# TimD1/vcfdist

Hardware: AMD Instinct MI355X
Metric: supercluster-alignments/sec (higher is better)
Workload: dtype int32; 1 GPU; wgs_synth; superclusters_per_gpu=1000000, span_dist=lognormal(median 20, sigma 1.2) clip [4,10000]

## Files before the change

### vcfdist_amd/csrc/pr_api.hip

```cpp
#include <hip/hip_runtime.h>
#include <hip/hip_ext.h>
#include <dlfcn.h>

#include <algorithm>
#include <atomic>
#include <chrono>
#include <cstdarg>
#include <cstdio>
#include <cstdlib>
#include <cstring>
#include <condition_variable>
#include <deque>
#include <functional>
#include <mutex>
#include <string>
#include <thread>
#include <tuple>
#include <unordered_map>
#include <unordered_set>
#include <vector>

#include "../../include/vcfdist_pr.h"
#include "pr_device.h"
#include "pr_plan.h"
// ... 734 lines not shown
        const int64_t D1_FLOOR = int64_t(4) << 20;
        const int64_t slack = 64 * 5 * int64_t(len_max + 1);
        const int64_t in_all = 2 * in_chunk_max + slack, log_all = 2 * log_max + 160 * int64_t((n_short_max + 63) / 64) + 160 * int64_t(len_max + 1);
        h->d1_in_cap = std::min(in_all, std::max(int64_t(D1_SHARE * double(in_all)), D1_FLOOR + slack));
        h->d1_log_cap = std::min(log_all, std::max(int64_t(D1_SHARE * double(log_all)), D1_FLOOR + slack));
        const int64_t cap_ip = std::min<int64_t>(n_short_max, std::max<int64_t>(4096, (n_short_max / 4 + 3) & ~int64_t(3)));
        h->d1_wave_cap = int32_t((cap_ip + 63) / 64);
        h->d1_fail_cap = int32_t(n_short_max + n_short_max / 8 + 1024);
        h->soft_alloc = true;
        int rc = dev_alloc(h, &h->d_d1_hdr, size_t(h->d1_wave_cap));
        if (!rc) rc = dev_alloc(h, &h->d_d1_in, size_t(h->d1_in_cap));
        if (!rc) rc = dev_alloc(h, &h->d_d1_log, size_t(h->d1_log_cap));
        if (!rc) rc = dev_alloc(h, &h->d_d1_fail, size_t(h->d1_fail_cap));
        if (!rc) rc = dev_alloc(h, &h->d_d1_info, 16);
        if (!rc) rc = dev_alloc(h, &h->d_d1_blk, size_t(h->d1_fail_cap / 256 + 8));
        h->soft_alloc = false;
        if (rc) {
            if (h->debug) fprintf(stderr, "[vpr] distance-1 lane level: no room for its blocks (%.2f GB), the level is off for this batch\n",
                                  double(h->d1_in_cap) * 4e-9 + double(h->d1_log_cap) * 16e-9);
            h->d_d1_hdr = nullptr; h->d_d1_in = nullptr; h->d_d1_log = nullptr; h->d_d1_fail = nullptr; h->d_d1_info = nullptr; h->d_d1_blk = nullptr;
            h->err.clear();
            (void)hipGetLastError();
        } else {
            HIPCHK(h, hipMemsetAsync(h->d_d1_info, 0, 64, h->stream));
        }
    }
    for (size_t ci = 0; ci < P.chunks.size(); ci++) {
        const Chunk &ch = P.chunks[ci];
        const int64_t n_short = ch.count - ch.n_long;
        if (n_short <= 0) continue;
        hipLaunchKernelGGL(k_prep_zl, dim3(unsigned((n_short + 63) / 64)), dim3(256), 0, h->stream, h->dB, h->d_descs,
                           P.d_work + ch.work_off + ch.n_long, int(n_short), h->d_zl_hdr + h->zl_wave0[ci], h->d_zl_in);
    }
    HIPCHK(h, hipGetLastError());
    if (h->debug) fprintf(stderr, "[vpr] zero-distance lane level: %zu waves, %.2f GB position words, %.2f GB log\n", n_waves,
                          double(in_words) * 4e-9, double(log_max) * 16e-9);
    return VPR_OK;
}

// ... 288 lines not shown
            VPRCHK(dev_alloc(h, &D.cand2_r[q], ref_len));
            VPRCHK(dev_alloc(h, &D.fk_q[q], hap_len[q]));
            VPRCHK(dev_alloc(h, &D.fk_r[q], ref_len));
            VPRCHK(dev_alloc(h, &D.bk_q[q], hap_len[q]));
            VPRCHK(dev_alloc(h, &D.bk_r[q], ref_len));
            VPRCHK(dev_alloc(h, &D.vs_ref[q], ref_len));
            VPRCHK(dev_alloc(h, &D.fk4_q[q], hap_len[q]));
            VPRCHK(dev_alloc(h, &D.fk4_r[q], ref_len));
            VPRCHK(dev_alloc(h, &D.tk[q], hap_len[2 + q]));
            VPRCHK(dev_alloc(h, &D.tj[q], hap_len[2 + q] + 8));
            VPRCHK(dev_alloc(h, &D.wk_q[q], hap_len[q]));
            VPRCHK(dev_alloc(h, &D.wk_r[q], ref_len));
            VPRCHK(dev_alloc(h, &D.wk_t[q], hap_len[2 + q]));
            VPRCHK(dev_alloc(h, &D.xb_q[q], hap_len[q]));
            VPRCHK(dev_alloc(h, &D.xb_r[q], ref_len));
            HIPCHK(h, hipMemsetAsync(D.cand_q[q], 0xff, std::max<int64_t>(hap_len[q], 1) * sizeof(int4), h->stream));
            HIPCHK(h, hipMemsetAsync(D.cand_r[q], 0xff, std::max<int64_t>(ref_len, 1) * sizeof(int4), h->stream));
            HIPCHK(h, hipMemsetAsync(D.cand2_q[q], 0xff, std::max<int64_t>(hap_len[q], 1) * sizeof(int4), h->stream));
            HIPCHK(h, hipMemsetAsync(D.cand2_r[q], 0xff, std::max<int64_t>(ref_len, 1) * sizeof(int4), h->stream));
        }
        lap("  inputs: reference arrays, constants' blocks");
        VPRCHK(dev_alloc(h, &h->d_err, 1));
        HIPCHK(h, hipMemsetAsync(h->d_err, 0, 4, h->stream));
        if (!h->ev_offsets) HIPCHK(h, hipEventCreateWithFlags(&h->ev_offsets, hipEventDisableTiming));
        HIPCHK(h, hipEventRecord(h->ev_offsets, h->stream));
        return VPR_OK;
    }

    int generate() {
        if (!h->gen_src) return VPR_OK;
// ... 45 lines not shown
    }

    template <typename K, typename... A>
    void query_planes(K kernel, A... tail) {
        for (int q = 0; q < 2; q++) {
            if (hap_len[q] > 0) hipLaunchKernelGGL(kernel, blocks(hap_len[q]), dim3(256), 0, h->stream, D, q, 0, hap_len[q], tail...);
            if (ref_len > 0) hipLaunchKernelGGL(kernel, blocks(ref_len), dim3(256), 0, h->stream, D, q, 1, ref_len, tail...);
        }
    }

    int prep_kernels() {
        for (hipEvent_t &e : ev_prep) HIPCHK(h, hipEventCreate(&e));
        HIPCHK(h, hipEventRecord(ev_prep[0], h->stream));
        if (n > 0) hipLaunchKernelGGL(k_prep_scof, dim3(unsigned((n + 255) / 256), 5), dim3(256), 0, h->stream, D);
        query_planes(k_prep_cand, h->d_err);
        query_planes(k_prep_pack);
        lap("  prep: scof, cand, pack");
        for (int s = 0; s < 4; s++)
            if (hap_len[s] > 0)
                hipLaunchKernelGGL(k_prep_ins, blocks(hap_len[s]), dim3(256), 0, h->stream, D, s, hap_len[s]);
        if (n > 0) hipLaunchKernelGGL(k_prep_suffix, dim3((n + 4 * SUFFIX_SC_PER_WAVE - 1) / (4 * SUFFIX_SC_PER_WAVE), 6), dim3(256), 0, h->stream, D);
        int2 *pd = nullptr;
        VPRCHK(pin_array(h, &pd, size_t(std::max(n, 1)) * 4));
        for (int s = 0; s < 4; s++) {
            h->hp_dspan[s] = pd + size_t(s) * size_t(n);
            if (n > 0) HIPCHK(h, hipMemcpyAsync(h->hp_dspan[s], D.dspan[s], size_t(n) * sizeof(int2), hipMemcpyDeviceToHost, h->stream));
        }
        lap("  prep: ins, suffix, spans");
        query_planes(k_prep_xb);
        for (int s = 0; s < 2; s++)
            if (hap_len[2 + s] > 0) hipLaunchKernelGGL(k_prep_tj, blocks(hap_len[2 + s]), dim3(256), 0, h->stream, D, s, hap_len[2 + s]);
        for (int w = 0; w < 6; w++) {
            const int64_t npos = w < 2 ? hap_len[w] : (w < 4 ? ref_len : hap_len[w - 2]);
            if (npos > 0) hipLaunchKernelGGL(k_prep_q16, blocks(npos), dim3(256), 0, h->stream, D, w, npos);
            if (npos > 0) hipLaunchKernelGGL(k_prep_wk, blocks(npos), dim3(256), 0, h->stream, D, w, npos);
        }
        HIPCHK(h, hipEventRecord(ev_prep[1], h->stream));
        return VPR_OK;
    }

    int batch_pass() {
        h->descs.set(b, h->var_off);
        h->ed_max_len = -1;
        na = h->descs.size();
        for (int s = 0; s < 4; s++) sec_total += 2 * b->var_off[s][n];
        sec_total += 16 * int64_t(n);
        const bool plan_pass = lv0 <= LV_Q16 && !(h->cfg.flags & VPR_CFG_HAP_DEDUP) && n > 0;
        const int LLT = h->long_lt;
        h->p0 = vpr_handle::Plan0Pass();
        if (plan_pass) h->level.resize(size_t(n) * 4);
// ... 1205 lines not shown
    void ordered_fails(const int32_t *list, int32_t nc, int32_t *out, int32_t *cnt, const int32_t *n_dev, hipStream_t ks) {
        const int nb = (nc + 255) / 256;
        hipLaunchKernelGGL(k_fails_count, dim3(nb), dim3(256), 0, ks, list, nc, h->d_outs, h->d_d1_blk, 1, n_dev);
        hipLaunchKernelGGL(k_fails_scan, dim3(1), dim3(FAILS_SCAN_NT), 0, ks, h->d_d1_blk, nb, cnt);
        hipLaunchKernelGGL(k_fails_scatter, dim3(nb), dim3(256), 0, ks, list, nc, h->d_outs, h->d_d1_blk, out, 1, n_dev);
    }

    int enqueue_d1(const int32_t *list, const int32_t *n_dev, int32_t cap, int32_t n_all, hipStream_t ks, int ph, int ztag) {
        const int nw = (cap + 63) / 64;
        vpr_launch_stat ls;
        memset(&ls, 0, sizeof(ls));
        ls.threads = 64; ls.cells_per_thread = 1; ls.n_units = cap;
        int rc = VPR_OK;
        if (ph == 1) {
            rc = timed(0, ls, ks, "k_prep_d1", [&] {
                hipLaunchKernelGGL(k_d1_hdr, dim3(nw), dim3(64), 0, ks, h->d_descs, list, n_dev, cap, h->d_outs, h->d_d1_hdr);
                hipLaunchKernelGGL(k_d1_scan, dim3(1), dim3(D1_SCAN_NT), 0, ks, h->d_d1_hdr, nw, h->d1_in_cap, h->d1_log_cap, h->d_d1_info);
                hipLaunchKernelGGL(k_prep_d1, dim3(nw), dim3(256), 0, ks, h->dB, h->d_descs, list, n_dev, cap, h->d_outs, h->d_d1_hdr, h->d_d1_in);
            });
            if (rc) return rc;
            rc = timed(1, ls, ks, "k_one_lane", [&] {
                hipLaunchKernelGGL(k_one_lane, dim3(nw), dim3(64), 0, ks, h->d_descs, list, n_dev, cap, h->d_d1_hdr, h->d_d1_in, h->d_d1_log,
                                   h->d_outs, reinterpret_cast<PathEnt *>(h->plan0.arena), (h->cfg.flags & VPR_CFG_KEEP_PATHS) ? 1 : 0, h->d_d1_info,
                                   std::max(1, h->lane_prio_rows / 4));
                hipLaunchKernelGGL(k_fwd_band_finish, dim3((cap + 255) / 256), dim3(256), 0, ks, list, cap, h->d_outs, D1_TAG, n_dev);
            });
            if (rc) return rc;
            ordered_fails(list, n_all, h->d_d1_fail, h->d_d1_info + 2, n_dev, ks);
        } else if (ph == 4) {
            ls.cells_per_thread = 3;
            rc = timed(3, ls, ks, "k_one_tail", [&] {
                hipLaunchKernelGGL(k_one_tail, dim3(nw), dim3(64), 0, ks, h->dB, h->d_descs, list, n_dev, cap, h->d_d1_hdr, h->d_d1_in, h->d_d1_log,
                                   h->d_outs, reinterpret_cast<PathEnt *>(h->plan0.arena), (h->cfg.flags & VPR_CFG_KEEP_PATHS) ? 1 : 0, h->d_d1_info,
// ... 399 lines not shown
                for (int ph = 1; ph <= 4; ph <<= 1) {
                    if ((rc = enqueue_part(P0, P0.d_work, ch.work_off + n_long, n_short, P0.lv, s_short, 1, n_long, false,
                                           ch.part_cells[1], ch.part_in[1], ch.part_dense[1], -1, ph))) return rc;
                    if (ph == 1) post_flag(1, s_short);
                    if (ph == 2 && (rc = collect_part(1, short_list, n_short, s_short))) return rc;
                }
            }
            if (inplace) {
                zl_wave0 = h->zl_wave0[ci];
                zl_rows = ch.part_rows[1];
                const int32_t *n_dev = h->d_cnt + 1;
                const int ztag = LV_TAG[LV_Z];
                HIPCHK(h, hipMemsetAsync(h->d_cnt + SLOT_IP, 0, 4, s_short));
                const bool d1 = h->d_d1_hdr != nullptr && cap_ip <= h->d1_wave_cap * 64;
                const int32_t n_all1 = n_short + n_short / 16 + 64;
                if (d1) HIPCHK(h, hipMemsetAsync(h->d_d1_info + 2, 0, 4, s_short));
                hipStream_t s_cred = h->side_credit ? h->cls_stream[7] : s_short;
                for (int ph = 1; ph <= 4; ph <<= 1) {
                    if (ph != 4 || s_cred == s_short) {
                        if ((rc = enqueue_part(P0, P0.d_work, ch.work_off + n_long, n_short, LV_Z, s_short, 1, n_long, false,
                                               ch.part_cells[1], ch.part_in[1], ch.part_dense[1], -1, ph))) return rc;
                        if (d1 && (rc = enqueue_d1(h->d_fail + n_long, n_dev, cap_ip, n_all1, s_short, ph, ztag))) return rc;
                    }
                    if (ph == 1 && s_cred != s_short) {
                        HIPCHK(h, hipEventRecord(h->ev_cred[0], s_short));
                        HIPCHK(h, hipStreamWaitEvent(s_cred, h->ev_cred[0], 0));
                        if ((rc = enqueue_part(P0, P0.d_work, ch.work_off + n_long, n_short, LV_Z, s_cred, 1, n_long, false,
                                               ch.part_cells[1], ch.part_in[1], ch.part_dense[1], -1, 4))) return rc;
                        if (d1 && (rc = enqueue_d1(h->d_fail + n_long, n_dev, cap_ip, n_all1, s_cred, 4, ztag))) return rc;
                        HIPCHK(h, hipEventRecord(h->ev_cred[1], s_cred));
                    }
// ... 505 lines not shown
```

### vcfdist_amd/csrc/pr_d1.hip

```cpp
#ifndef PR_D1_HIP_
#define PR_D1_HIP_

#define D1_TAG 9
#define D1_CLEAN ZL_CLEAN_REJECT

#define GE_ALIVE 1u
#define GE_MAT 2u
#define GE_SWP 4u
#define GE_PSLOT_SHIFT 3
#define GE_SUB 32u
#define GE_SUB_SHIFT 6
#define GE_INS 256u
#define GE_INS_SHIFT 9
#define GE_DEL 2048u
#define GE_DEL_SHIFT 12
#define GE_TP 16384u
#define GE_BWD 32768u

#define MV_SWP_R 0
#define MV_MAT 1
#define MV_SUB 2
#define MV_INS 3
#define MV_DEL 4
#define MV_SWP_Q 5

__global__ void __launch_bounds__(64) k_d1_hdr(const AlnDesc *__restrict__ descs, const int32_t *__restrict__ list,
                                               const int32_t *__restrict__ n_dev, int n_cap, const AlnOut *__restrict__ outs,
                                               ZlWave *__restrict__ hdr) {
    const int w = blockIdx.x, lane = threadIdx.x;
    const int n = min(*n_dev, n_cap);
    const int wi = w * 64 + lane;
    const int a = wi < n ? list[wi] : -1;
    int lq = 0, lr = 0, lt = 0;
    if (a >= 0 && outs[a].exit_min == D1_CLEAN) {
        const AlnDesc *d = descs + a;
        lq = d->Lq; lr = d->Lr; lt = d->Lt;
    }
#pragma unroll
    for (int o = 32; o; o >>= 1) {
        lq = max(lq, __shfl_xor(lq, o)); lr = max(lr, __shfl_xor(lr, o)); lt = max(lt, __shfl_xor(lt, o));
    }
    if (lane == 0) {
        ZlWave W;
        W.in_off = 0; W.log_off = 0; W.mq = lq; W.mr = lr; W.mt = lt; W.pad = 0;
        hdr[w] = W;
    }
}

#define D1_SCAN_NT 256
__global__ void __launch_bounds__(D1_SCAN_NT) k_d1_scan(ZlWave *__restrict__ hdr, int n_waves, int64_t in_cap, int64_t log_cap,
                                                  int32_t *__restrict__ info) {
    __shared__ int64_t s_in[D1_SCAN_NT], s_log[D1_SCAN_NT];
    __shared__ int s_used, s_drop;
    const int tid = threadIdx.x;
    if (tid == 0) { s_used = 0; s_drop = 0; }
    const int per = (n_waves + D1_SCAN_NT - 1) / D1_SCAN_NT;
    const int b = min(n_waves, tid * per), e = min(n_waves, b + per);
    int64_t si = 0, sl = 0;
    for (int k = b; k < e; k++) {
        const ZlWave W = hdr[k];
        if (W.mt > 0) { si += 64 * (2 * int64_t(W.mq) + 2 * int64_t(W.mr) + W.mt); sl += 160 * (int64_t(W.mt) + 1); }
    }
    s_in[tid] = si; s_log[tid] = sl;
    __syncthreads();
    for (int o = 1; o < D1_SCAN_NT; o <<= 1) {
        const int64_t ai = tid >= o ? s_in[tid - o] : 0, al = tid >= o ? s_log[tid - o] : 0;
        __syncthreads();
        s_in[tid] += ai; s_log[tid] += al;
        __syncthreads();
    }
    int64_t oi = s_in[tid] - si, ol = s_log[tid] - sl;
    int used = 0, drop = 0;
    for (int k = b; k < e; k++) {
        ZlWave W = hdr[k];
        if (W.mt <= 0) continue;
        const int64_t ni = 64 * (2 * int64_t(W.mq) + 2 * int64_t(W.mr) + W.mt), nl = 160 * (int64_t(W.mt) + 1);
        if (oi + ni > in_cap || ol + nl > log_cap) { W.mq = W.mr = W.mt = 0; drop++; }
        else { W.in_off = oi; W.log_off = ol; used++; }
        oi += ni; ol += nl;
        hdr[k] = W;
    }
    if (used) atomicAdd(&s_used, used);
    if (drop) atomicAdd(&s_drop, drop);
    __syncthreads();
    if (tid == 0) { info[0] = s_used; info[1] = s_drop; }
}

__global__ void __launch_bounds__(256) k_prep_d1(DevBatch B, const AlnDesc *__restrict__ descs, const int32_t *__restrict__ list,
                                                 const int32_t *__restrict__ n_dev, int n_cap, const AlnOut *__restrict__ outs,
                                                 const ZlWave *__restrict__ hdr, uint32_t *__restrict__ zin) {
    __shared__ uint32_t tile[64][65];
    __shared__ int64_t s_qo[64], s_ro[64], s_to[64];
    __shared__ int32_t s_lq[64], s_lr[64], s_lt[64];
    __shared__ uint8_t s_qs[64], s_ts[64];
    const int w = blockIdx.x;
    const ZlWave H = hdr[w];
    if (H.mt <= 0) return;
    const int n_list = min(*n_dev, n_cap);
    const int lane = threadIdx.x & 63, sub = threadIdx.x >> 6;
    if (threadIdx.x < 64) {
        const int wi = w * 64 + lane;
        int a = wi < n_list ? list[wi] : -1;
        if (a >= 0 && outs[a].exit_min != D1_CLEAN) a = -1;
        if (a >= 0) {
            const AlnDesc *d = descs + a;
            s_qo[lane] = d->q_off; s_ro[lane] = d->r_off; s_to[lane] = d->t_off;
            s_lq[lane] = d->Lq; s_lr[lane] = d->Lr; s_lt[lane] = d->Lt;
            s_qs[lane] = uint8_t(d->qs); s_ts[lane] = uint8_t(d->ts);
        } else {
            s_qo[lane] = s_ro[lane] = s_to[lane] = 0;
            s_lq[lane] = s_lr[lane] = s_lt[lane] = 0;
            s_qs[lane] = 0; s_ts[lane] = 2;
        }
    }
    __syncthreads();
    auto flagbits = [](int f) -> uint32_t { return ((f & PV) ? ZW_PV : 0u) | ((f & PB) ? ZW_PB : 0u) | ((f & PE) ? ZW_PE : 0u); };
    uint32_t *out = zin + H.in_off;
    for (int arr = 0; arr < 5; arr++) {
        const int pl = arr >> 1;
        const bool src_words = (arr & 1) && arr < 4;
        const int mlen = pl == 0 ? H.mq : (pl == 1 ? H.mr : H.mt);
        for (int x0 = 0; x0 < mlen; x0 += 64) {
            const int x = x0 + lane;
#pragma unroll 16
            for (int k = 0; k < 16; k++) {
                const int l = sub * 16 + k;
                const int qs = s_qs[l], ts = s_ts[l];
                const int Lr = s_lr[l];
                const int len = pl == 0 ? s_lq[l] : (pl == 1 ? Lr : s_lt[l]);
                uint32_t v = src_words ? 0u : 0x7f0000u;
                if (x < len) {
                    const int64_t ro = s_ro[l];
                    if (src_words) {
                        const int4 c = pl == 0 ? B.cand_q[qs][s_qo[l] + x] : B.cand_r[qs][ro + x];
                        v = uint32_t(c.x >= 0 ? c.x + 1 : 0) | (c.z >= 0 ? 0xffff0000u : (uint32_t(c.y >= 0 ? c.y + 1 : 0) << 16));
                    } else {
                        const int slot = pl == 2 ? ts : qs;
                        const int64_t o = (pl == 0 ? s_qo[l] : (pl == 1 ? ro : s_to[l])) + x;
                        const uint8_t *seq = pl == 1 ? B.ref_seq : B.hap_seq[slot];
                        const int2 *wk = pl == 0 ? B.wk_q[qs] : (pl == 1 ? B.wk_r[qs] : B.wk_t[ts - 2]);
                        const int2 k2 = wk[o];
                        const int p = k2.x, f = pl == 1 ? int(B.ref_flag[qs][o]) : (k2.y & 0xff);
                        const uint32_t ins = ((k2.y >> 8) & ((1 << qs) | (1 << ts))) ? ZW_INS : 0u;
                        v = uint32_t((p + 1) & 0xffff) | (uint32_t(seq[o] & 0x7f) << 16) | flagbits(f) | ins;
                        if (pl == 0 && x > 0 && ((p != wk[o - 1].x + 1) || (f & PB))) v |= ZW_TP;
                        (void)Lr;
                    }
                }
                tile[lane][l] = v;
            }
            __syncthreads();
            const int rows = min(64, mlen - x0);
            for (int r = sub; r < rows; r += 4) out[int64_t(x0 + r) * 64 + lane] = tile[r][lane];
            __syncthreads();
        }
        out += int64_t(mlen) * 64;
    }
}

__global__ void __launch_bounds__(64, 3) k_one_lane(const AlnDesc *__restrict__ descs, const int32_t *__restrict__ list,
                                                    const int32_t *__restrict__ n_dev, int n_cap, const ZlWave *__restrict__ hdr,
                                                    const uint32_t *__restrict__ zin, uint4 *__restrict__ zlog,
                                                    AlnOut *__restrict__ outs, PathEnt *__restrict__ paths, int keep_paths,
                                                    int32_t *__restrict__ info, int prio_rows) {
    const int w = blockIdx.x, lane = threadIdx.x;
    const ZlWave H = hdr[w];
    if (H.mt <= 0) return;
    if (H.mt >= prio_rows) __builtin_amdgcn_s_setprio(2);
    const int n_list = min(*n_dev, n_cap);
    const int wi = w * 64 + lane;
    int a_ = wi < n_list ? list[wi] : -1;
    if (a_ >= 0 && outs[a_].exit_min != D1_CLEAN) a_ = -1;
// ... 586 lines not shown
```

### vcfdist_amd/csrc/pr_device.h

```cpp
#ifndef PR_DEVICE_H_
#define PR_DEVICE_H_
#include <hip/hip_runtime.h>
#include <stdint.h>

#define F_INS 1
#define F_DEL 2
#define F_MAT 4
#define F_SUB 8
#define F_SWP 16
#define F_CHOICE_SHIFT 5
#define F_TIE 128
#define F_CHOICE_MASK (0x60u | F_SUB)
__host__ __device__ __forceinline__ uint32_t f_choice_bits(int rank) { return (uint32_t(rank & 3) << F_CHOICE_SHIFT) | (uint32_t(rank >> 2) << 3); }
__host__ __device__ __forceinline__ int f_choice_of(uint32_t f) { return int(((f >> F_CHOICE_SHIFT) & 3u) | ((f >> 1) & 4u)); }
__host__ __device__ __forceinline__ uint32_t f_diag(uint32_t f) { return f & (F_MAT | (F_SUB & ~(f >> 1))); }
__host__ __device__ __forceinline__ uint32_t rank_bits(int rank) { return (uint32_t(rank & 3) << 1) | (uint32_t(rank >> 2) << 4); }
__host__ __device__ __forceinline__ int rank_of(uint32_t bits) { return int(((bits >> 1) & 3u) | ((bits >> 2) & 4u)); }
#define F_SWP_KEY_MASK (F_SWP | F_CHOICE_MASK)
__host__ __device__ __forceinline__ uint32_t f_swp_key(int rank) { return F_SWP | f_choice_bits(rank); }
#define SWAP_SOURCES_MAX 8
#define F_KEEP 0xe0

#define PV 1
#define PB 2
// ... 30 lines not shown
    int2 *fk_r[2];
    int32_t *bk_q[2];
    int32_t *bk_r[2];
    int32_t *vs_hap[4];
    int32_t *vs_ref[2];
    int2 *xb_q[2];
    int2 *xb_r[2];
    int2 *dspan[4];
    int4 *fk4_q[2];
    int4 *fk4_r[2];
    int2 *tk[2];
    uint16_t *tj[2];
    int2 *wk_q[2];
    int2 *wk_r[2];
    int2 *wk_t[2];
};
#define FK_MULTI (1 << 30)
#define FK_NONE24 0xffffff

struct AlnDesc {
    int64_t q_off, t_off, r_off;
    int32_t Lq, Lt, Lr;
    int32_t qs, ts;
    int32_t sc, aln;
    int32_t pitch[2];
    int64_t mat_off[2];
    int64_t path_off;
    int64_t sec_off;
    int32_t sec_cap;
    int32_t path_cap;
// ... 131 lines not shown
```

### vcfdist_amd/csrc/pr_host.h

```cpp
#ifndef PR_HOST_H_
#define PR_HOST_H_
#include <hip/hip_runtime.h>
#include <hip/hip_ext.h>

#include <algorithm>
#include <atomic>
#include <chrono>
#include <cstdarg>
#include <cstdio>
#include <cstdlib>
#include <cstring>
#include <condition_variable>
#include <deque>
#include <functional>
#include <mutex>
#include <string>
#include <thread>
#include <tuple>
#include <unordered_map>
#include <unordered_set>
#include <vector>

#include "../../include/vcfdist_pr.h"
#include "pr_device.h"
// ... 270 lines not shown
    EdJob *d_jobs = nullptr; int32_t jobs_cap = 0; int32_t *d_njobs = nullptr;
    uint32_t *d_err = nullptr;
    int32_t *d_fail = nullptr, *d_cnt = nullptr;
    int4 *d_tie_list = nullptr, *hp_tie_list = nullptr; int32_t tie_list_cap = 0;
    int32_t *hp_flag = nullptr; int32_t flag_seq = 0;
    int32_t *d_tie_cnt = nullptr, *hp_tie_cnt = nullptr;
    hipEvent_t ev_spec = nullptr;
    TieJob *hp_tie_jobs = nullptr; size_t tie_jobs_cap = 0;
    int4 *d_tie_dec = nullptr; int64_t tie_dec_cap = 0;
    int32_t *d_tie_ndec = nullptr;
    std::vector<int32_t> plan0_pos;
    ZlWave *d_zl_hdr = nullptr; uint32_t *d_zl_in = nullptr; uint4 *d_zl_log = nullptr;
    std::vector<int64_t> zl_wave0;
    ZlWave *d_d1_hdr = nullptr; uint32_t *d_d1_in = nullptr; uint4 *d_d1_log = nullptr; int32_t *d_d1_fail = nullptr, *d_d1_info = nullptr;
    int32_t *d_d1_blk = nullptr;
    hipEvent_t ev_offsets = nullptr;
    hipEvent_t ev_cred[2] = {nullptr, nullptr};
    bool side_credit = true;
    struct Plan0Pass {
        bool valid = false, bad = false;
        int64_t part_cells[2] = {0, 0}, part_in[2] = {0, 0}, part_dense[2] = {0, 0}, part_rows[2] = {0, 0}, need128 = 0, need_max = 0;
        std::vector<std::pair<int64_t, int32_t>> big;
    } p0;
    int64_t d1_in_cap = 0, d1_log_cap = 0;
    int32_t d1_wave_cap = 0, d1_fail_cap = 0;
    int32_t d1_max_rows = 256;
    std::vector<ZlWave> zl_hdr_host;
    int32_t long_lt = LONG_LT;
    const vpr_variants *gen_src = nullptr;
    uint8_t *d_ctg_seq = nullptr; const uint8_t *ctg_src = nullptr; int64_t ctg_bytes = 0; uint64_t ctg_probe = 0;
// ... 166 lines not shown
```

### vcfdist_amd/csrc/pr_mem.hip

```cpp
#include "pr_host.h"

namespace {
std::string g_create_err;
}
const char *vpr_create_error() { return g_create_err.c_str(); }

int fail(vpr_handle *h, int code, const char *fmt, ...) {
    char buf[512];
    va_list ap;
    va_start(ap, fmt);
    vsnprintf(buf, sizeof(buf), fmt, ap);
    va_end(ap);
    if (h) h->err = buf; else g_create_err = buf;
    return code;
}


inline void slow_call(vpr_handle *h, const char *what, const char *site, size_t bytes, double dt) {
    if (h && h->stall_log && dt > 5.0) fprintf(stderr, "[vpr] slow host call: %s (%zu bytes) at %s: %.1f ms\n", what, bytes, site, dt);
}
const char *exp_getenv(const char *name) {
#ifdef VPR_EXPERIMENTS
    return getenv(name);
#else
// ... 269 lines not shown
            keep.tie_scratch[e] = h->lad[k].tie_scratch[e]; keep.tie_scratch_bytes[e] = h->lad[k].tie_scratch_bytes[e];
            keep.tie_first[e] = h->lad[k].tie_first[e];
        }
        h->lad[k] = keep;
    }
    for (auto &b : h->parked) h->dev_cache.push_back(b);
    h->parked.clear();
    h->resident.clear();
    h->res0_cnt = 0;
    h->d_ed_scratch = nullptr; h->ed_scratch_ints = 0;
    h->d_tie_list = nullptr; h->hp_tie_list = nullptr; h->tie_list_cap = 0; h->d_tie_cnt = nullptr; h->hp_tie_cnt = nullptr;
    h->hp_tie_jobs = nullptr; h->tie_jobs_cap = 0;
    h->d_tie_dec = nullptr; h->tie_dec_cap = 0; h->d_tie_ndec = nullptr; h->plan0_pos.clear();
    h->d_zl_hdr = nullptr; h->d_zl_in = nullptr; h->d_zl_log = nullptr; h->zl_wave0.clear();
    h->d_d1_hdr = nullptr; h->d_d1_in = nullptr; h->d_d1_log = nullptr; h->d_d1_fail = nullptr; h->d_d1_info = nullptr; h->d_d1_blk = nullptr;
    h->d1_in_cap = h->d1_log_cap = 0; h->d1_wave_cap = h->d1_fail_cap = 0;
    h->uploaded = h->executed = false;
}

int64_t books_free(int64_t reported_free, int64_t total) { return dev_books().books_free(reported_free, total); }
```

### vcfdist_amd/csrc/pr_zl.hip

```cpp
#ifndef PR_ZL_HIP_
#define PR_ZL_HIP_
#include <type_traits>


#define ZW_PTR(w) (int((w) & 0xffffu) - 1)
#define ZW_BASE(w) (((w) >> 16) & 0x7fu)
#define ZW_PV (1u << 23)
#define ZW_PB (1u << 24)
#define ZW_PE (1u << 25)
#define ZW_INS (1u << 26)
#define ZW_TP (1u << 27)
__device__ __forceinline__ bool zw_fwd_allow(uint32_t w) { return !(w & ZW_PV) || (w & ZW_PE); }
__device__ __forceinline__ bool zw_bwd_allow(uint32_t w) { return !(w & ZW_PV) || (w & ZW_PB); }

#define ZE_ALIVE 1u
#define ZE_HASMAT 2u
#define ZE_HASSWP 4u
#define ZE_PSLOT_SHIFT 3
#define ZE_TP 32u
#define ZE_BWD 64u

#define ZL_MAXLEN 65000
#define ZL_CLEAN_REJECT (-1)

__global__ void __launch_bounds__(256) k_prep_zl(DevBatch B, const AlnDesc *__restrict__ descs, const int32_t *__restrict__ list,
                                                 int n_list, const ZlWave *__restrict__ hdr, uint32_t *__restrict__ zin) {
    __shared__ uint32_t tile[64][65];
    __shared__ int64_t s_qo[64], s_ro[64], s_to[64];
    __shared__ int32_t s_lq[64], s_lr[64], s_lt[64];
    __shared__ uint8_t s_qs[64], s_ts[64];
    const int w = blockIdx.x;
    const ZlWave H = hdr[w];
    const int lane = threadIdx.x & 63, sub = threadIdx.x >> 6;
    if (threadIdx.x < 64) {
        const int wi = w * 64 + lane;
        const int a = wi < n_list ? list[wi] : -1;
        if (a >= 0) {
            const AlnDesc *d = descs + a;
            s_qo[lane] = d->q_off; s_ro[lane] = d->r_off; s_to[lane] = d->t_off;
            s_lq[lane] = d->Lq; s_lr[lane] = d->Lr; s_lt[lane] = d->Lt;
            s_qs[lane] = uint8_t(d->qs); s_ts[lane] = uint8_t(d->ts);
        } else {
            s_qo[lane] = s_ro[lane] = s_to[lane] = 0;
            s_lq[lane] = s_lr[lane] = s_lt[lane] = 0;
            s_qs[lane] = 0; s_ts[lane] = 2;
        }
    }
    __syncthreads();
    auto flagbits = [](int f) -> uint32_t { return ((f & PV) ? ZW_PV : 0u) | ((f & PB) ? ZW_PB : 0u) | ((f & PE) ? ZW_PE : 0u); };
    uint32_t *out = zin + H.in_off;
    for (int arr = 0; arr < 3; arr++) {
        const int mlen = arr == 0 ? H.mq : (arr == 1 ? H.mr : H.mt);
        for (int x0 = 0; x0 < mlen; x0 += 64) {
            const int x = x0 + lane;
#pragma unroll 16
            for (int k = 0; k < 16; k++) {
                const int l = sub * 16 + k;
                const int qs = s_qs[l], ts = s_ts[l];
                const int Lr = s_lr[l];
                const int len = arr == 0 ? s_lq[l] : (arr == 1 ? Lr : s_lt[l]);
                uint32_t v = 0x7f0000u;
                if (x < len) {
                    const int64_t ro = s_ro[l];
                    const int slot = arr == 2 ? ts : qs;
                    const int64_t o = (arr == 0 ? s_qo[l] : (arr == 1 ? ro : s_to[l])) + x;
                    const uint8_t *seq = arr == 1 ? B.ref_seq : B.hap_seq[slot];
                    const int2 *wk = arr == 0 ? B.wk_q[qs] : (arr == 1 ? B.wk_r[qs] : B.wk_t[ts - 2]);
                    const int2 k2 = wk[o];
                    const int p = k2.x, f = arr == 1 ? int(B.ref_flag[qs][o]) : (k2.y & 0xff);
                    const uint32_t ins = ((k2.y >> 8) & ((1 << qs) | (1 << ts))) ? ZW_INS : 0u;
                    v = uint32_t((p + 1) & 0xffff) | (uint32_t(seq[o] & 0x7f) << 16) | flagbits(f) | ins;
                    if (arr == 0 && x > 0 && ((p != wk[o - 1].x + 1) || (f & PB))) v |= ZW_TP;
                    (void)Lr;
                }
                tile[lane][l] = v;
            }
            __syncthreads();
            const int rows = min(64, mlen - x0);
            for (int r = sub; r < rows; r += 4) out[int64_t(x0 + r) * 64 + lane] = tile[r][lane];
            __syncthreads();
        }
        out += int64_t(mlen) * 64;
    }
}

typedef __attribute__((ext_vector_type(4))) unsigned int zl_u4;
typedef __attribute__((ext_vector_type(2))) unsigned int zl_u2;
#define ZL_OOB 0xfffffff0u

__global__ void __launch_bounds__(64, 6) k_zero_lane(const AlnDesc *__restrict__ descs, const int32_t *__restrict__ list, int n_list,
                                                  const ZlWave *__restrict__ hdr, const uint32_t *__restrict__ zin,
                                                  uint4 *__restrict__ zlog, AlnOut *__restrict__ outs, PathEnt *__restrict__ paths,
                                                  int keep_paths, int d1_max_rows, int prio_rows) {
    const int w = blockIdx.x, lane = threadIdx.x;
    const ZlWave H = hdr[w];
    if (H.mt >= prio_rows) __builtin_amdgcn_s_setprio(2);
    const int wi = w * 64 + lane;
    const int a_ = wi < n_list ? list[wi] : -1;
// ... 362 lines not shown
```

Baseline: 201.2 million supercluster-alignments/s.

## Precompute packed lane words and fuse distance-1 header, scan and prep into one kernel

Adds per-position prep kernels (k_prep_zw, k_prep_zs) that precompute packed 32-bit lane words once, so the zero- and distance-1 transposes gather one word per position instead of reassembling from several arrays. Both transposes now share a software-pipelined transpose helper that overlaps the next tile's loads with the current tile's stores and writes via buffer stores. The separate header, single-block scan and prep kernels for distance-1 are merged into one kernel that uses a ticket counter and a decoupled look-back prefix sum. This trades extra device memory and prep passes, plus spin-wait risk, for fewer launches and less serialized scan work.

```diff
diff --git a/vcfdist_amd/csrc/pr_api.hip b/vcfdist_amd/csrc/pr_api.hip
--- a/vcfdist_amd/csrc/pr_api.hip
+++ b/vcfdist_amd/csrc/pr_api.hip
@@ -772,15 +772,20 @@
         if (!rc) rc = dev_alloc(h, &h->d_d1_fail, size_t(h->d1_fail_cap));
         if (!rc) rc = dev_alloc(h, &h->d_d1_info, 16);
         if (!rc) rc = dev_alloc(h, &h->d_d1_blk, size_t(h->d1_fail_cap / 256 + 8));
+        const size_t scan_words = D1_SCAN_HEAD + 4 * size_t(h->d1_wave_cap);
+        if (!rc) rc = dev_alloc(h, &h->d_d1_scan, scan_words);
         h->soft_alloc = false;
         if (rc) {
             if (h->debug) fprintf(stderr, "[vpr] distance-1 lane level: no room for its blocks (%.2f GB), the level is off for this batch\n",
                                   double(h->d1_in_cap) * 4e-9 + double(h->d1_log_cap) * 16e-9);
             h->d_d1_hdr = nullptr; h->d_d1_in = nullptr; h->d_d1_log = nullptr; h->d_d1_fail = nullptr; h->d_d1_info = nullptr; h->d_d1_blk = nullptr;
+            h->d_d1_scan = nullptr;
             h->err.clear();
             (void)hipGetLastError();
         } else {
             HIPCHK(h, hipMemsetAsync(h->d_d1_info, 0, 64, h->stream));
+            HIPCHK(h, hipMemsetAsync(h->d_d1_scan, 0, scan_words * 8, h->stream));
+            h->d1_tickets = 0; h->d1_gen = 0;
         }
     }
     for (size_t ci = 0; ci < P.chunks.size(); ci++) {
@@ -1099,6 +1104,11 @@
             VPRCHK(dev_alloc(h, &D.wk_t[q], hap_len[2 + q]));
             VPRCHK(dev_alloc(h, &D.xb_q[q], hap_len[q]));
             VPRCHK(dev_alloc(h, &D.xb_r[q], ref_len));
+            VPRCHK(dev_alloc(h, &D.zw_q[q], hap_len[q]));
+            VPRCHK(dev_alloc(h, &D.zw_r[q], ref_len));
+            VPRCHK(dev_alloc(h, &D.zw_t[q], hap_len[2 + q]));
+            VPRCHK(dev_alloc(h, &D.zs_q[q], hap_len[q]));
+            VPRCHK(dev_alloc(h, &D.zs_r[q], ref_len));
             HIPCHK(h, hipMemsetAsync(D.cand_q[q], 0xff, std::max<int64_t>(hap_len[q], 1) * sizeof(int4), h->stream));
             HIPCHK(h, hipMemsetAsync(D.cand_r[q], 0xff, std::max<int64_t>(ref_len, 1) * sizeof(int4), h->stream));
             HIPCHK(h, hipMemsetAsync(D.cand2_q[q], 0xff, std::max<int64_t>(hap_len[q], 1) * sizeof(int4), h->stream));
@@ -1174,6 +1184,7 @@
         HIPCHK(h, hipEventRecord(ev_prep[0], h->stream));
         if (n > 0) hipLaunchKernelGGL(k_prep_scof, dim3(unsigned((n + 255) / 256), 5), dim3(256), 0, h->stream, D);
         query_planes(k_prep_cand, h->d_err);
+        query_planes(k_prep_zs);
         query_planes(k_prep_pack);
         lap("  prep: scof, cand, pack");
         for (int s = 0; s < 4; s++)
@@ -1194,6 +1205,7 @@
             const int64_t npos = w < 2 ? hap_len[w] : (w < 4 ? ref_len : hap_len[w - 2]);
             if (npos > 0) hipLaunchKernelGGL(k_prep_q16, blocks(npos), dim3(256), 0, h->stream, D, w, npos);
             if (npos > 0) hipLaunchKernelGGL(k_prep_wk, blocks(npos), dim3(256), 0, h->stream, D, w, npos);
+            if (npos > 0) hipLaunchKernelGGL(k_prep_zw, blocks(npos), dim3(256), 0, h->stream, D, w, npos);
         }
         HIPCHK(h, hipEventRecord(ev_prep[1], h->stream));
         return VPR_OK;
@@ -2429,9 +2441,9 @@
         int rc = VPR_OK;
         if (ph == 1) {
             rc = timed(0, ls, ks, "k_prep_d1", [&] {
-                hipLaunchKernelGGL(k_d1_hdr, dim3(nw), dim3(64), 0, ks, h->d_descs, list, n_dev, cap, h->d_outs, h->d_d1_hdr);
-                hipLaunchKernelGGL(k_d1_scan, dim3(1), dim3(D1_SCAN_NT), 0, ks, h->d_d1_hdr, nw, h->d1_in_cap, h->d1_log_cap, h->d_d1_info);
-                hipLaunchKernelGGL(k_prep_d1, dim3(nw), dim3(256), 0, ks, h->dB, h->d_descs, list, n_dev, cap, h->d_outs, h->d_d1_hdr, h->d_d1_in);
+                hipLaunchKernelGGL(k_prep_d1, dim3(nw), dim3(256), 0, ks, h->dB, h->d_descs, list, n_dev, cap, h->d_outs, h->d_d1_hdr, nw,
+                                   h->d_d1_in, h->d_d1_scan, h->d1_tickets, ++h->d1_gen, h->d1_in_cap, h->d1_log_cap, h->d_d1_info);
+                h->d1_tickets += (unsigned long long)nw;
             });
             if (rc) return rc;
             rc = timed(1, ls, ks, "k_one_lane", [&] {
@@ -2861,7 +2873,7 @@
                 HIPCHK(h, hipMemsetAsync(h->d_cnt + SLOT_IP, 0, 4, s_short));
                 const bool d1 = h->d_d1_hdr != nullptr && cap_ip <= h->d1_wave_cap * 64;
                 const int32_t n_all1 = n_short + n_short / 16 + 64;
-                if (d1) HIPCHK(h, hipMemsetAsync(h->d_d1_info + 2, 0, 4, s_short));
+                if (d1) HIPCHK(h, hipMemsetAsync(h->d_d1_info, 0, 12, s_short));
                 hipStream_t s_cred = h->side_credit ? h->cls_stream[7] : s_short;
                 for (int ph = 1; ph <= 4; ph <<= 1) {
                     if (ph != 4 || s_cred == s_short) {
diff --git a/vcfdist_amd/csrc/pr_d1.hip b/vcfdist_amd/csrc/pr_d1.hip
--- a/vcfdist_amd/csrc/pr_d1.hip
+++ b/vcfdist_amd/csrc/pr_d1.hip
@@ -24,138 +24,106 @@
 #define MV_DEL 4
 #define MV_SWP_Q 5
 
-__global__ void __launch_bounds__(64) k_d1_hdr(const AlnDesc *__restrict__ descs, const int32_t *__restrict__ list,
-                                               const int32_t *__restrict__ n_dev, int n_cap, const AlnOut *__restrict__ outs,
-                                               ZlWave *__restrict__ hdr) {
-    const int w = blockIdx.x, lane = threadIdx.x;
-    const int n = min(*n_dev, n_cap);
-    const int wi = w * 64 + lane;
-    const int a = wi < n ? list[wi] : -1;
-    int lq = 0, lr = 0, lt = 0;
-    if (a >= 0 && outs[a].exit_min == D1_CLEAN) {
-        const AlnDesc *d = descs + a;
-        lq = d->Lq; lr = d->Lr; lt = d->Lt;
-    }
-#pragma unroll
-    for (int o = 32; o; o >>= 1) {
-        lq = max(lq, __shfl_xor(lq, o)); lr = max(lr, __shfl_xor(lr, o)); lt = max(lt, __shfl_xor(lt, o));
-    }
-    if (lane == 0) {
+#define D1_SCAN_HEAD 4
+#define D1_SPIN_MAX (1 << 16)
+typedef unsigned long long d1_u64;
+__device__ __forceinline__ void d1_publish(d1_u64 *g, uint32_t gen, uint32_t v) {
+    __hip_atomic_store(g, (d1_u64(gen) << 32) | v, __ATOMIC_RELAXED, __HIP_MEMORY_SCOPE_AGENT);
+}
+__device__ __forceinline__ bool d1_lookback(d1_u64 *gran, int w, uint32_t gen, int lane, uint32_t &ex_in, uint32_t &ex_log) {
+    d1_u64 si = 0, sl = 0;
+    for (int base = w - 1; base >= 0; base -= 64) {
+        const int idx = base - lane;
+        int state = 2;
+        uint32_t vi = 0, vl = 0;
+        if (idx >= 0) {
+            d1_u64 *g = gran + 4 * int64_t(idx);
+            state = 0;
+            for (int spins = 0; spins < D1_SPIN_MAX; spins++) {
+                const d1_u64 pi = __hip_atomic_load(g + 2, __ATOMIC_RELAXED, __HIP_MEMORY_SCOPE_AGENT);
+                const d1_u64 pl = __hip_atomic_load(g + 3, __ATOMIC_RELAXED, __HIP_MEMORY_SCOPE_AGENT);
+                if (uint32_t(pi >> 32) == gen && uint32_t(pl >> 32) == gen) { state = 2; vi = uint32_t(pi); vl = uint32_t(pl); break; }
+                const d1_u64 ai = __hip_atomic_load(g + 0, __ATOMIC_RELAXED, __HIP_MEMORY_SCOPE_AGENT);
+                const d1_u64 al = __hip_atomic_load(g + 1, __ATOMIC_RELAXED, __HIP_MEMORY_SCOPE_AGENT);
+                if (uint32_t(ai >> 32) == gen && uint32_t(al >> 32) == gen) { state = 1; vi = uint32_t(ai); vl = uint32_t(al); break; }
+                __builtin_amdgcn_s_sleep(2);
+            }
+        }
+        if (__any(state == 0)) return false;
+        const d1_u64 pm = __ballot(state == 2);
+        const int j = pm ? __ffsll(pm) - 1 : 64;
+        d1_u64 ti = lane <= j ? vi : 0u, tl = lane <= j ? vl : 0u;
+#pragma unroll
+        for (int o = 32; o; o >>= 1) { ti += __shfl_xor(ti, o); tl += __shfl_xor(tl, o); }
+        si += ti; sl += tl;
+        if (j < 64) break;
+    }
+    ex_in = uint32_t(min(si, d1_u64(0xffffffffu))); ex_log = uint32_t(min(sl, d1_u64(0xffffffffu)));
+    return true;
+}
+
+__global__ void __launch_bounds__(256, 8) k_prep_d1(DevBatch B, const AlnDesc *__restrict__ descs, const int32_t *__restrict__ list,
+                                                 const int32_t *__restrict__ n_dev, int n_cap, const AlnOut *__restrict__ outs,
+                                                 ZlWave *__restrict__ hdr, int n_waves, uint32_t *__restrict__ zin,
+                                                 d1_u64 *__restrict__ scan, d1_u64 ticket0, uint32_t gen, int64_t in_cap,
+                                                 int64_t log_cap, int32_t *__restrict__ info) {
+    __shared__ ZlTurn<5> S;
+    __shared__ ZlWave s_H;
+    if (threadIdx.x < 64) {
+        const int lane = threadIdx.x;
+        d1_u64 tk = 0;
+        if (lane == 0) tk = atomicAdd(scan, d1_u64(1)) - ticket0;
+        tk = __shfl(tk, 0);
         ZlWave W;
-        W.in_off = 0; W.log_off = 0; W.mq = lq; W.mr = lr; W.mt = lt; W.pad = 0;
-        hdr[w] = W;
-    }
-}
-
-#define D1_SCAN_NT 256
-__global__ void __launch_bounds__(D1_SCAN_NT) k_d1_scan(ZlWave *__restrict__ hdr, int n_waves, int64_t in_cap, int64_t log_cap,
-                                                  int32_t *__restrict__ info) {
-    __shared__ int64_t s_in[D1_SCAN_NT], s_log[D1_SCAN_NT];
-    __shared__ int s_used, s_drop;
-    const int tid = threadIdx.x;
-    if (tid == 0) { s_used = 0; s_drop = 0; }
-    const int per = (n_waves + D1_SCAN_NT - 1) / D1_SCAN_NT;
-    const int b = min(n_waves, tid * per), e = min(n_waves, b + per);
-    int64_t si = 0, sl = 0;
-    for (int k = b; k < e; k++) {
-        const ZlWave W = hdr[k];
-        if (W.mt > 0) { si += 64 * (2 * int64_t(W.mq) + 2 * int64_t(W.mr) + W.mt); sl += 160 * (int64_t(W.mt) + 1); }
-    }
-    s_in[tid] = si; s_log[tid] = sl;
+        W.in_off = 0; W.log_off = 0; W.mq = 0; W.mr = 0; W.mt = 0; W.pad = 0;
+        if (tk < d1_u64(n_waves)) {
+            const int w = int(tk);
+            const int n = min(*n_dev, n_cap);
+            const int wi = w * 64 + lane;
+            int a = wi < n ? list[wi] : -1;
+            if (a >= 0 && outs[a].exit_min != D1_CLEAN) a = -1;
+            int lq = 0, lr = 0, lt = 0;
+            if (a >= 0) {
+                const AlnDesc *d = descs + a;
+                const int qs = d->qs, ts = d->ts;
+                lq = d->Lq; lr = d->Lr; lt = d->Lt;
+                S.ptr[0][lane] = zl_gptr(B.zw_q[qs] + d->q_off); S.ptr[1][lane] = zl_gptr(B.zs_q[qs] + d->q_off);
+                S.ptr[2][lane] = zl_gptr(B.zw_r[qs] + d->r_off); S.ptr[3][lane] = zl_gptr(B.zs_r[qs] + d->r_off);
+                S.ptr[4][lane] = zl_gptr(B.zw_t[ts - 2] + d->t_off);
+                S.slots[lane] = (1u << qs) | (1u << ts);
+            } else {
+                for (int k = 0; k < 5; k++) S.ptr[k][lane] = zl_gptr(scan);
+                S.slots[lane] = 0;
+            }
+            S.len[0][lane] = lq; S.len[1][lane] = lr; S.len[2][lane] = lt;
+#pragma unroll
+            for (int o = 32; o; o >>= 1) {
+                lq = max(lq, __shfl_xor(lq, o)); lr = max(lr, __shfl_xor(lr, o)); lt = max(lt, __shfl_xor(lt, o));
+            }
+            d1_u64 *g = scan + D1_SCAN_HEAD + 4 * int64_t(w);
+            const uint32_t ni = lt > 0 ? uint32_t(2 * lq + 2 * lr + lt) : 0u, nl = lt > 0 ? uint32_t(lt + 1) : 0u;
+            if (lane == 0) { d1_publish(g + 0, gen, ni); d1_publish(g + 1, gen, nl); }
+            if (lt > 0) {
+                uint32_t ei = 0, el = 0;
+                const bool ok = d1_lookback(scan + D1_SCAN_HEAD, w, gen, lane, ei, el);
+                if (ok && lane == 0) { d1_publish(g + 2, gen, uint32_t(min(d1_u64(ei) + ni, d1_u64(0xffffffffu)))); d1_publish(g + 3, gen, uint32_t(min(d1_u64(el) + nl, d1_u64(0xffffffffu)))); }
+                const int64_t oi = 64 * int64_t(ei), ol = 160 * int64_t(el);
+                if (!ok || oi + 64 * int64_t(ni) > in_cap || ol + 160 * int64_t(nl) > log_cap) {
+                    if (lane == 0) atomicAdd(info + 1, 1);
+                } else {
+                    W.in_off = oi; W.log_off = ol; W.mq = lq; W.mr = lr; W.mt = lt;
+                    if (lane == 0) atomicAdd(info + 0, 1);
+                }
+            }
+            if (lane == 0) hdr[w] = W;
+        }
+        if (lane == 0) s_H = W;
+    }
     __syncthreads();
-    for (int o = 1; o < D1_SCAN_NT; o <<= 1) {
-        const int64_t ai = tid >= o ? s_in[tid - o] : 0, al = tid >= o ? s_log[tid - o] : 0;
-        __syncthreads();
-        s_in[tid] += ai; s_log[tid] += al;
-        __syncthreads();
-    }
-    int64_t oi = s_in[tid] - si, ol = s_log[tid] - sl;
-    int used = 0, drop = 0;
-    for (int k = b; k < e; k++) {
-        ZlWave W = hdr[k];
-        if (W.mt <= 0) continue;
-        const int64_t ni = 64 * (2 * int64_t(W.mq) + 2 * int64_t(W.mr) + W.mt), nl = 160 * (int64_t(W.mt) + 1);
-        if (oi + ni > in_cap || ol + nl > log_cap) { W.mq = W.mr = W.mt = 0; drop++; }
-        else { W.in_off = oi; W.log_off = ol; used++; }
-        oi += ni; ol += nl;
-        hdr[k] = W;
-    }
-    if (used) atomicAdd(&s_used, used);
-    if (drop) atomicAdd(&s_drop, drop);
-    __syncthreads();
-    if (tid == 0) { info[0] = s_used; info[1] = s_drop; }
-}
-
-__global__ void __launch_bounds__(256) k_prep_d1(DevBatch B, const AlnDesc *__restrict__ descs, const int32_t *__restrict__ list,
-                                                 const int32_t *__restrict__ n_dev, int n_cap, const AlnOut *__restrict__ outs,
-                                                 const ZlWave *__restrict__ hdr, uint32_t *__restrict__ zin) {
-    __shared__ uint32_t tile[64][65];
-    __shared__ int64_t s_qo[64], s_ro[64], s_to[64];
-    __shared__ int32_t s_lq[64], s_lr[64], s_lt[64];
-    __shared__ uint8_t s_qs[64], s_ts[64];
-    const int w = blockIdx.x;
-    const ZlWave H = hdr[w];
+    const ZlWave H = s_H;
     if (H.mt <= 0) return;
-    const int n_list = min(*n_dev, n_cap);
-    const int lane = threadIdx.x & 63, sub = threadIdx.x >> 6;
-    if (threadIdx.x < 64) {
-        const int wi = w * 64 + lane;
-        int a = wi < n_list ? list[wi] : -1;
-        if (a >= 0 && outs[a].exit_min != D1_CLEAN) a = -1;
-        if (a >= 0) {
-            const AlnDesc *d = descs + a;
-            s_qo[lane] = d->q_off; s_ro[lane] = d->r_off; s_to[lane] = d->t_off;
-            s_lq[lane] = d->Lq; s_lr[lane] = d->Lr; s_lt[lane] = d->Lt;
-            s_qs[lane] = uint8_t(d->qs); s_ts[lane] = uint8_t(d->ts);
-        } else {
-            s_qo[lane] = s_ro[lane] = s_to[lane] = 0;
-            s_lq[lane] = s_lr[lane] = s_lt[lane] = 0;
-            s_qs[lane] = 0; s_ts[lane] = 2;
-        }
-    }
-    __syncthreads();
-    auto flagbits = [](int f) -> uint32_t { return ((f & PV) ? ZW_PV : 0u) | ((f & PB) ? ZW_PB : 0u) | ((f & PE) ? ZW_PE : 0u); };
-    uint32_t *out = zin + H.in_off;
-    for (int arr = 0; arr < 5; arr++) {
-        const int pl = arr >> 1;
-        const bool src_words = (arr & 1) && arr < 4;
-        const int mlen = pl == 0 ? H.mq : (pl == 1 ? H.mr : H.mt);
-        for (int x0 = 0; x0 < mlen; x0 += 64) {
-            const int x = x0 + lane;
-#pragma unroll 16
-            for (int k = 0; k < 16; k++) {
-                const int l = sub * 16 + k;
-                const int qs = s_qs[l], ts = s_ts[l];
-                const int Lr = s_lr[l];
-                const int len = pl == 0 ? s_lq[l] : (pl == 1 ? Lr : s_lt[l]);
-                uint32_t v = src_words ? 0u : 0x7f0000u;
-                if (x < len) {
-                    const int64_t ro = s_ro[l];
-                    if (src_words) {
-                        const int4 c = pl == 0 ? B.cand_q[qs][s_qo[l] + x] : B.cand_r[qs][ro + x];
-                        v = uint32_t(c.x >= 0 ? c.x + 1 : 0) | (c.z >= 0 ? 0xffff0000u : (uint32_t(c.y >= 0 ? c.y + 1 : 0) << 16));
-                    } else {
-                        const int slot = pl == 2 ? ts : qs;
-                        const int64_t o = (pl == 0 ? s_qo[l] : (pl == 1 ? ro : s_to[l])) + x;
-                        const uint8_t *seq = pl == 1 ? B.ref_seq : B.hap_seq[slot];
-                        const int2 *wk = pl == 0 ? B.wk_q[qs] : (pl == 1 ? B.wk_r[qs] : B.wk_t[ts - 2]);
-                        const int2 k2 = wk[o];
-                        const int p = k2.x, f = pl == 1 ? int(B.ref_flag[qs][o]) : (k2.y & 0xff);
-                        const uint32_t ins = ((k2.y >> 8) & ((1 << qs) | (1 << ts))) ? ZW_INS : 0u;
-                        v = uint32_t((p + 1) & 0xffff) | (uint32_t(seq[o] & 0x7f) << 16) | flagbits(f) | ins;
-                        if (pl == 0 && x > 0 && ((p != wk[o - 1].x + 1) || (f & PB))) v |= ZW_TP;
-                        (void)Lr;
-                    }
-                }
-                tile[lane][l] = v;
-            }
-            __syncthreads();
-            const int rows = min(64, mlen - x0);
-            for (int r = sub; r < rows; r += 4) out[int64_t(x0 + r) * 64 + lane] = tile[r][lane];
-            __syncthreads();
-        }
-        out += int64_t(mlen) * 64;
-    }
+    const int mlen[5] = {H.mq, H.mq, H.mr, H.mr, H.mt};
+    zl_turn<5, 0xau, 0x250u>(S, mlen, zin + H.in_off);
 }
 
 __global__ void __launch_bounds__(64, 3) k_one_lane(const AlnDesc *__restrict__ descs, const int32_t *__restrict__ list,
diff --git a/vcfdist_amd/csrc/pr_device.h b/vcfdist_amd/csrc/pr_device.h
--- a/vcfdist_amd/csrc/pr_device.h
+++ b/vcfdist_amd/csrc/pr_device.h
@@ -68,6 +68,11 @@
     int2 *wk_q[2];
     int2 *wk_r[2];
     int2 *wk_t[2];
+    uint32_t *zw_q[2];
+    uint32_t *zw_r[2];
+    uint32_t *zw_t[2];
+    uint32_t *zs_q[2];
+    uint32_t *zs_r[2];
 };
 #define FK_MULTI (1 << 30)
 #define FK_NONE24 0xffffff
diff --git a/vcfdist_amd/csrc/pr_host.h b/vcfdist_amd/csrc/pr_host.h
--- a/vcfdist_amd/csrc/pr_host.h
+++ b/vcfdist_amd/csrc/pr_host.h
@@ -308,6 +308,7 @@
     std::vector<int64_t> zl_wave0;
     ZlWave *d_d1_hdr = nullptr; uint32_t *d_d1_in = nullptr; uint4 *d_d1_log = nullptr; int32_t *d_d1_fail = nullptr, *d_d1_info = nullptr;
     int32_t *d_d1_blk = nullptr;
+    unsigned long long *d_d1_scan = nullptr, d1_tickets = 0; uint32_t d1_gen = 0;
     hipEvent_t ev_offsets = nullptr;
     hipEvent_t ev_cred[2] = {nullptr, nullptr};
     bool side_credit = true;
diff --git a/vcfdist_amd/csrc/pr_mem.hip b/vcfdist_amd/csrc/pr_mem.hip
--- a/vcfdist_amd/csrc/pr_mem.hip
+++ b/vcfdist_amd/csrc/pr_mem.hip
@@ -307,6 +307,7 @@
     h->d_tie_dec = nullptr; h->tie_dec_cap = 0; h->d_tie_ndec = nullptr; h->plan0_pos.clear();
     h->d_zl_hdr = nullptr; h->d_zl_in = nullptr; h->d_zl_log = nullptr; h->zl_wave0.clear();
     h->d_d1_hdr = nullptr; h->d_d1_in = nullptr; h->d_d1_log = nullptr; h->d_d1_fail = nullptr; h->d_d1_info = nullptr; h->d_d1_blk = nullptr;
+    h->d_d1_scan = nullptr; h->d1_tickets = 0; h->d1_gen = 0;
     h->d1_in_cap = h->d1_log_cap = 0; h->d1_wave_cap = h->d1_fail_cap = 0;
     h->uploaded = h->executed = false;
 }
diff --git a/vcfdist_amd/csrc/pr_zl.hip b/vcfdist_amd/csrc/pr_zl.hip
--- a/vcfdist_amd/csrc/pr_zl.hip
+++ b/vcfdist_amd/csrc/pr_zl.hip
@@ -23,65 +23,126 @@
 #define ZL_MAXLEN 65000
 #define ZL_CLEAN_REJECT (-1)
 
-__global__ void __launch_bounds__(256) k_prep_zl(DevBatch B, const AlnDesc *__restrict__ descs, const int32_t *__restrict__ list,
+__global__ void k_prep_zw(DevBatch B, int which, int64_t n_pos) {
+    const int64_t g = int64_t(blockIdx.x) * blockDim.x + threadIdx.x;
+    if (g >= n_pos) return;
+    int2 k2;
+    int f, base;
+    if (which < 2) { k2 = B.wk_q[which][g]; f = k2.y & 0xff; base = B.hap_seq[which][g]; }
+    else if (which < 4) { k2 = B.wk_r[which - 2][g]; f = int(B.ref_flag[which - 2][g]); base = B.ref_seq[g]; }
+    else { k2 = B.wk_t[which - 4][g]; f = k2.y & 0xff; base = B.hap_seq[which - 2][g]; }
+    const int p = k2.x;
+    uint32_t v = uint32_t((p + 1) & 0xffff) | (uint32_t(base & 0x7f) << 16) | ((f & PV) ? ZW_PV : 0u) | ((f & PB) ? ZW_PB : 0u) |
+                 ((f & PE) ? ZW_PE : 0u) | (uint32_t((k2.y >> 8) & 0xf) << 28);
+    if (which < 2) {
+        const int64_t beg = B.hap_off[which][B.sc_hap[which][g]];
+        if (g > beg && ((p != B.wk_q[which][g - 1].x + 1) || (f & PB))) v |= ZW_TP;
+        B.zw_q[which][g] = v;
+    } else if (which < 4) {
+        B.zw_r[which - 2][g] = v;
+    } else {
+        B.zw_t[which - 4][g] = v;
+    }
+}
+__device__ __forceinline__ uint32_t zl_fold(uint32_t v, uint32_t slots) {
+    return (v & 0x0fffffffu) | (((v >> 28) & slots) ? ZW_INS : 0u);
+}
+
+__global__ void k_prep_zs(DevBatch B, int h, int dir, int64_t n_pos) {
+    const int64_t g = int64_t(blockIdx.x) * blockDim.x + threadIdx.x;
+    if (g >= n_pos) return;
+    const int4 c = dir == 0 ? B.cand_q[h][g] : B.cand_r[h][g];
+    const uint32_t v = uint32_t(c.x >= 0 ? c.x + 1 : 0) | (c.z >= 0 ? 0xffff0000u : (uint32_t(c.y >= 0 ? c.y + 1 : 0) << 16));
+    (dir == 0 ? B.zs_q[h] : B.zs_r[h])[g] = v;
+}
+
+typedef const __attribute__((address_space(1))) uint32_t *zl_gptr;
+template <int NA>
+struct ZlTurn {
+    zl_gptr ptr[NA][64];
+    int32_t len[3][64];
+    uint32_t slots[64];
+    uint32_t tile[64][65];
+};
+template <int NA, uint32_t SRC, uint32_t PL>
+__device__ __forceinline__ void zl_turn(ZlTurn<NA> &S, const int (&mlen)[NA], uint32_t *__restrict__ out) {
+    const int lane = threadIdx.x & 63, sub = threadIdx.x >> 6;
+    struct It { int a, x0; int64_t base; };
+    auto settle = [&](It &i) { while (i.a < NA && i.x0 >= mlen[i.a]) { i.base += int64_t(mlen[i.a]) * 64; i.a++; i.x0 = 0; } };
+    auto request = [&](const It &i, uint32_t (&v)[16]) -> uint32_t {
+        const int x = i.x0 + lane;
+        const int pl = int((PL >> (2 * i.a)) & 3u);
+        uint32_t in = 0;
+#pragma unroll
+        for (int k = 0; k < 16; k++) {
+            const int l = sub * 16 + k;
+            const bool on = x < S.len[pl][l];
+            in |= uint32_t(on) << k;
+            v[k] = S.ptr[i.a][l][on ? x : 0];
+        }
+        return in;
+    };
+    It cur{0, 0, 0};
+    settle(cur);
+    if (cur.a >= NA) return;
+    int64_t words = 0;
+#pragma unroll
+    for (int a = 0; a < NA; a++) words += int64_t(mlen[a]) * 64;
+    const auto rout = __builtin_amdgcn_make_buffer_rsrc(out, 0, int(words * 4), 0x00020000);
+    uint64_t slots16 = 0;
+#pragma unroll
+    for (int k = 0; k < 16; k++) slots16 |= uint64_t(S.slots[sub * 16 + k] & 0xfu) << (4 * k);
+    uint32_t v[16];
+    uint32_t in = request(cur, v);
+    while (cur.a < NA) {
+        const bool src = (SRC >> cur.a) & 1u;
+#pragma unroll
+        for (int k = 0; k < 16; k++) {
+            const int l = sub * 16 + k;
+            const bool on = (in >> k) & 1u;
+            const uint32_t word = zl_fold(v[k], uint32_t(slots16 >> (4 * k)) & 0xfu);
+            S.tile[lane][l] = src ? (on ? v[k] : 0u) : (on ? word : 0x7f0000u);
+        }
+        It nxt = cur;
+        nxt.x0 += 64;
+        settle(nxt);
+        if (nxt.a < NA) in = request(nxt, v);
+        lds_barrier<256>();
+        const int rows = min(64, mlen[cur.a] - cur.x0);
+        const uint32_t row0 = uint32_t(cur.base + int64_t(cur.x0) * 64 + sub * 64 + lane) << 2;
+#pragma unroll
+        for (int i = 0; i < 16; i++) {
+            const int r = sub + 4 * i;
+            __builtin_amdgcn_raw_buffer_store_b32(S.tile[r][lane], rout, r < rows ? row0 + uint32_t(i) * 1024u : 0xfffffff0u, 0, 0);
+        }
+        lds_barrier<256>();
+        cur = nxt;
+    }
+}
+
+__global__ void __launch_bounds__(256, 8) k_prep_zl(DevBatch B, const AlnDesc *__restrict__ descs, const int32_t *__restrict__ list,
                                                  int n_list, const ZlWave *__restrict__ hdr, uint32_t *__restrict__ zin) {
-    __shared__ uint32_t tile[64][65];
-    __shared__ int64_t s_qo[64], s_ro[64], s_to[64];
-    __shared__ int32_t s_lq[64], s_lr[64], s_lt[64];
-    __shared__ uint8_t s_qs[64], s_ts[64];
+    __shared__ ZlTurn<3> S;
     const int w = blockIdx.x;
     const ZlWave H = hdr[w];
-    const int lane = threadIdx.x & 63, sub = threadIdx.x >> 6;
     if (threadIdx.x < 64) {
+        const int lane = threadIdx.x;
         const int wi = w * 64 + lane;
         const int a = wi < n_list ? list[wi] : -1;
         if (a >= 0) {
             const AlnDesc *d = descs + a;
-            s_qo[lane] = d->q_off; s_ro[lane] = d->r_off; s_to[lane] = d->t_off;
-            s_lq[lane] = d->Lq; s_lr[lane] = d->Lr; s_lt[lane] = d->Lt;
-            s_qs[lane] = uint8_t(d->qs); s_ts[lane] = uint8_t(d->ts);
+            const int qs = d->qs, ts = d->ts;
+            S.ptr[0][lane] = zl_gptr(B.zw_q[qs] + d->q_off); S.ptr[1][lane] = zl_gptr(B.zw_r[qs] + d->r_off); S.ptr[2][lane] = zl_gptr(B.zw_t[ts - 2] + d->t_off);
+            S.len[0][lane] = d->Lq; S.len[1][lane] = d->Lr; S.len[2][lane] = d->Lt;
+            S.slots[lane] = (1u << qs) | (1u << ts);
         } else {
-            s_qo[lane] = s_ro[lane] = s_to[lane] = 0;
-            s_lq[lane] = s_lr[lane] = s_lt[lane] = 0;
-            s_qs[lane] = 0; s_ts[lane] = 2;
+            for (int k = 0; k < 3; k++) { S.ptr[k][lane] = zl_gptr(hdr); S.len[k][lane] = 0; }
+            S.slots[lane] = 0;
         }
     }
     __syncthreads();
-    auto flagbits = [](int f) -> uint32_t { return ((f & PV) ? ZW_PV : 0u) | ((f & PB) ? ZW_PB : 0u) | ((f & PE) ? ZW_PE : 0u); };
-    uint32_t *out = zin + H.in_off;
-    for (int arr = 0; arr < 3; arr++) {
-        const int mlen = arr == 0 ? H.mq : (arr == 1 ? H.mr : H.mt);
-        for (int x0 = 0; x0 < mlen; x0 += 64) {
-            const int x = x0 + lane;
-#pragma unroll 16
-            for (int k = 0; k < 16; k++) {
-                const int l = sub * 16 + k;
-                const int qs = s_qs[l], ts = s_ts[l];
-                const int Lr = s_lr[l];
-                const int len = arr == 0 ? s_lq[l] : (arr == 1 ? Lr : s_lt[l]);
-                uint32_t v = 0x7f0000u;
-                if (x < len) {
-                    const int64_t ro = s_ro[l];
-                    const int slot = arr == 2 ? ts : qs;
-                    const int64_t o = (arr == 0 ? s_qo[l] : (arr == 1 ? ro : s_to[l])) + x;
-                    const uint8_t *seq = arr == 1 ? B.ref_seq : B.hap_seq[slot];
-                    const int2 *wk = arr == 0 ? B.wk_q[qs] : (arr == 1 ? B.wk_r[qs] : B.wk_t[ts - 2]);
-                    const int2 k2 = wk[o];
-                    const int p = k2.x, f = arr == 1 ? int(B.ref_flag[qs][o]) : (k2.y & 0xff);
-                    const uint32_t ins = ((k2.y >> 8) & ((1 << qs) | (1 << ts))) ? ZW_INS : 0u;
-                    v = uint32_t((p + 1) & 0xffff) | (uint32_t(seq[o] & 0x7f) << 16) | flagbits(f) | ins;
-                    if (arr == 0 && x > 0 && ((p != wk[o - 1].x + 1) || (f & PB))) v |= ZW_TP;
-                    (void)Lr;
-                }
-                tile[lane][l] = v;
-            }
-            __syncthreads();
-            const int rows = min(64, mlen - x0);
-            for (int r = sub; r < rows; r += 4) out[int64_t(x0 + r) * 64 + lane] = tile[r][lane];
-            __syncthreads();
-        }
-        out += int64_t(mlen) * 64;
-    }
+    const int mlen[3] = {H.mq, H.mr, H.mt};
+    zl_turn<3, 0u, 0x24u>(S, mlen, zin + H.in_off);
 }
 
 typedef __attribute__((ext_vector_type(4))) unsigned int zl_u4;
```

Result: no change. 200.1 million supercluster-alignments/s (-0.6%).
